# AIGC-Audio/AudioGPT

Hardware: AMD Instinct MI355X
Metric: generated audio-seconds/sec (10s clip, 100 DDIM steps) [3 independent batches of 8 prompts in flight per GPU] (higher is better)
Workload: dtype bf16x3; 1 GPU; Make-An-Audio T2A batch=8/GPU, 100 DDIM steps, CFG 1.5, UNet+VAE+HiFi-GAN(16k), fp32 storage, bf16x3-split MFMA (hi/lo, fp32 accumulate; meets the fp32 parity gates); prompts_per_gpu=8, ddim_steps=100, mel_frames=624, hipgraph=True, batches_in_flight=3, cfg_lanes=1, concurrency_hint=3, parallelism=prompt-sharded x1 (RCCL bcast cond / gather wav)

## Files before the change

### audiogpt_amd/csrc/igemm_dma.hip

```cpp
#include "igemm_epilogue.h"

#include <cstdio>
#include <cstdlib>

namespace maa {

namespace {

constexpr int NT = 256;

template <int BM, int BN, int WGM, int WGN, int NS, int TERMS>
__global__ __launch_bounds__(NT) void igemm_dma_kernel(const IGemm p, int ntiles, int Nb) {
    constexpr int WTM = BM / WGM, WTN = BN / WGN;
    constexpr int MI = WTM / 32, NI = WTN / 32;
    constexpr int ROWS = BM + BN;
    constexpr int STAGE = ROWS * 128;
    constexpr int IPW = ROWS / 32;
    static_assert(WGM * WGN == 4 && BM % 32 == 0 && BN % 32 == 0 && NS >= 2, "tile");
    static_assert((NS - 2) * IPW <= 63, "vmcnt field");
    extern __shared__ __attribute__((aligned(1024))) char smem[];

    const int tid = threadIdx.x;
    const int lane = tid & 63, wid = tid >> 6;
    const int bid = xcd_contiguous((int)blockIdx.x, (int)gridDim.x);
    const int nt = bid % ntiles, mt = bid / ntiles;
    const int m0 = mt * BM, n0 = nt * BN;

    const int Ctot = p.C1;
    const int rpb = p.Hout * p.Wout;
    const int Hlim = p.Hin << p.up, Wlim = p.Win << p.up;
    const int taps = p.KH * p.KW;
    const char* zero = reinterpret_cast<const char*>(p.zeros);

    bool is_a[IPW];
    int a_b[IPW], a_iy0[IPW], a_ix0[IPW];
    const char* a_slot[IPW];
    const char* src[IPW];
    bool ok[IPW];
#pragma unroll
    for (int j = 0; j < IPW; ++j) {
        const int row = 8 * (wid * IPW + j) + (lane >> 3);
        const int slot = (lane & 7) ^ ((row >> 1) & 7);
        is_a[j] = 8 * (wid * IPW + j) < BM;
        a_b[j] = -1;
        a_iy0[j] = a_ix0[j] = 0;
        a_slot[j] = reinterpret_cast<const char*>(p.a1) + slot * 16;
        src[j] = zero;
        ok[j] = false;
        if (is_a[j]) {
            const int m = m0 + row;
            if (m < p.M) {
                const int b = m / rpb;
                const int rem = m - b * rpb;
                const int oy = rem / p.Wout;
                a_b[j] = b;
                a_iy0[j] = oy * p.sh - p.ph;
                a_ix0[j] = (rem - oy * p.Wout) * p.sw - p.pw;
            }
        } else {
            const int n = n0 + row - BM;
            ok[j] = n < Nb;
            src[j] = reinterpret_cast<const char*>(p.b) + (long long)(ok[j] ? n : 0) * p.ldb * 4 + slot * 16;
        }
    }
    auto set_tap = [&](int tap) {
        const int ky = tap / p.KW, kx = tap - ky * p.KW;
#pragma unroll
        for (int j = 0; j < IPW; ++j)
            if (is_a[j]) {
                int iy = a_iy0[j] + ky * p.dh, ix = a_ix0[j] + kx * p.dw;
                const bool v = a_b[j] >= 0 && iy >= 0 && iy < Hlim && ix >= 0 && ix < Wlim;
                iy >>= p.up;
                ix >>= p.up;
                const long long off = v ? ((long long)a_b[j] * p.Hin + iy) * p.Win + ix : 0;
                ok[j] = v;
                src[j] = a_slot[j] + off * p.lda1 * 4;
            }
    };
    int g_tap = 0, g_ci = 0;
    bool past = false;
    auto issue = [&](int stage) {
        char* sbase = smem + stage * STAGE + wid * (IPW * 1024);
        const int k0 = g_tap * Ctot + g_ci;
#pragma unroll
        for (int j = 0; j < IPW; ++j) {
            const int off = is_a[j] ? g_ci : k0;
            const bool live = ok[j] && !past && (is_a[j] || k0 < p.K);
            const char* g = live ? src[j] + (long long)off * 4 : zero;
            __builtin_amdgcn_global_load_lds((gptr_t)g, (lptr_t)(sbase + j * 1024), 16, 0, 0);
        }
        g_ci += BK;
        if (g_ci >= Ctot) {
            g_ci = 0;
            ++g_tap;
            if (g_tap < taps)
                set_tap(g_tap);
            else
                past = true;
        }
    };

    f32x16 acc[MI][NI];
#pragma unroll
    for (int i = 0; i < MI; ++i)
#pragma unroll
        for (int j = 0; j < NI; ++j)
#pragma unroll
            for (int r = 0; r < 16; ++r) acc[i][j][r] = 0.f;

    const int wm = wid / WGN, wn = wid - wm * WGN;
    const int lrow = lane & 31, lk = lane >> 5;
    const int swz = (lrow >> 1) & 7;
    const int a_row = (wm * WTM + lrow) * 128, b_row = (BM + wn * WTN + lrow) * 128;
    int slot_off[2][2];
#pragma unroll
    for (int pl = 0; pl < 2; ++pl)
#pragma unroll
        for (int ks = 0; ks < 2; ++ks) slot_off[pl][ks] = ((pl * 4 + ks * 2 + lk) ^ swz) << 4;

    auto compute = [&](int stage) {
        const char* base = smem + stage * STAGE;
        constexpr int G = MI * NI == 1 ? 2 : 1;
#pragma unroll
        for (int k0 = 0; k0 < 2; k0 += G) {
            bf16x8 ah[G][MI], bh[G][NI], al[G][MI], bl[G][NI];
#pragma unroll
            for (int g = 0; g < G; ++g) {
                const int ks = k0 + g;
#pragma unroll
                for (int i = 0; i < MI; ++i)
                    if constexpr (TERMS == 3) al[g][i] = *reinterpret_cast<const bf16x8*>(base + a_row + i * 4096 + slot_off[1][ks]);
#pragma unroll
                for (int j = 0; j < NI; ++j) bh[g][j] = *reinterpret_cast<const bf16x8*>(base + b_row + j * 4096 + slot_off[0][ks]);
#pragma unroll
                for (int i = 0; i < MI; ++i) ah[g][i] = *reinterpret_cast<const bf16x8*>(base + a_row + i * 4096 + slot_off[0][ks]);
#pragma unroll
                for (int j = 0; j < NI; ++j)
                    if constexpr (TERMS == 3) bl[g][j] = *reinterpret_cast<const bf16x8*>(base + b_row + j * 4096 + slot_off[1][ks]);
            }
            __builtin_amdgcn_sched_barrier(0);
#pragma unroll
            for (int g = 0; g < G; ++g) {
                if constexpr (TERMS == 3) {
#pragma unroll
                    for (int i = 0; i < MI; ++i)
#pragma unroll
                        for (int j = 0; j < NI; ++j)
                            acc[i][j] = __builtin_amdgcn_mfma_f32_32x32x16_bf16(al[g][i], bh[g][j], acc[i][j], 0, 0, 0);
#pragma unroll
                    for (int i = 0; i < MI; ++i)
#pragma unroll
                        for (int j = 0; j < NI; ++j)
                            acc[i][j] = __builtin_amdgcn_mfma_f32_32x32x16_bf16(ah[g][i], bl[g][j], acc[i][j], 0, 0, 0);
                }
#pragma unroll
                for (int i = 0; i < MI; ++i)
#pragma unroll
                    for (int j = 0; j < NI; ++j)
                        acc[i][j] = __builtin_amdgcn_mfma_f32_32x32x16_bf16(ah[g][i], bh[g][j], acc[i][j], 0, 0, 0);
            }
        }
    };

    const int nchunks = (p.K + BK - 1) / BK;
    set_tap(0);
#pragma unroll
    for (int s = 0; s < NS - 1; ++s) issue(s);
    int st = 0, st_fill = NS - 1;
    for (int c = 0; c < nchunks; ++c) {
        wait_vmcnt<(NS - 2) * IPW>();
        __builtin_amdgcn_s_barrier();
        issue(st_fill);
        compute(st);
        st = st + 1 == NS ? 0 : st + 1;
        st_fill = st_fill + 1 == NS ? 0 : st_fill + 1;
    }
    wait_vmcnt<0>();

    igemm_epilogue<MI, NI>(p, acc, m0 + wm * WTM, n0 + wn * WTN, lrow, lk, 0, Nb, rpb);
}

template <int BM, int BN, int WGM, int WGN, int NS, int TERMS>
void launch_terms(const Ctx& ctx, const IGemm& p, int Nb) {
    const int ncols = p.N * (p.geglu ? 2 : 1);
    const int mtiles = (p.M + BM - 1) / BM, ntiles = (ncols + BN - 1) / BN;
    dim3 grid((unsigned)((long long)mtiles * ntiles));
    constexpr size_t lds = (size_t)NS * (BM + BN) * 128;
    auto kern = igemm_dma_kernel<BM, BN, WGM, WGN, NS, TERMS>;
    ensure_dynamic_lds(reinterpret_cast<const void*>(kern), ctx.device, (int)lds);
    hipLaunchKernelGGL(kern, grid, dim3(NT), lds, ctx.stream, p, ntiles, Nb);
}

template <int BM, int BN, int WGM, int WGN, int NS>
void launch_one(const Ctx& ctx, const IGemm& p, int Nb) {
    if (ctx.dtype == 2)
        launch_terms<BM, BN, WGM, WGN, NS, 1>(ctx, p, Nb);
    else
        launch_terms<BM, BN, WGM, WGN, NS, 3>(ctx, p, Nb);
}

}

bool igemm_dma_takes(const Ctx&, const IGemm& p, IGemmPlan& pl) {
    const long long ncols = (long long)p.N * (p.geglu ? 2 : 1);
    if (pl.cfg == 2 && p.K >= 1024 && ((p.M + 127) / 128) * ((ncols + 63) / 64) >= 448) pl.cfg = 1;
    pl.engine = IGemmPlan::DMA;
    return true;
}

void launch_igemm_dma(const Ctx& ctx, const IGemm& p, const IGemmPlan& pl) {
    const int cfg = pl.cfg, Nb = pl.Nb;
    const long long ncols = (long long)p.N * (p.geglu ? 2 : 1);
    int ns = cfg == 2 ? 2 : cfg == 1 ? 3 : 2;
    if (cfg == 2) {
        const long long tiles = (long long)((p.M + 63) / 64) * ((ncols + 63) / 64);
        if (tiles * 2 < 5LL * device_cu_count(ctx.device)) ns = 3;
    }
    switch (cfg) {
        case 0:
            launch_one<128, 128, 2, 2, 2>(ctx, p, Nb);
            break;
        case 1:
            launch_one<128, 64, 2, 2, 3>(ctx, p, Nb);
            break;
        default:
            if (ns >= 4) launch_one<64, 64, 2, 2, 4>(ctx, p, Nb);
            else if (ns == 3) launch_one<64, 64, 2, 2, 3>(ctx, p, Nb);
            else launch_one<64, 64, 2, 2, 2>(ctx, p, Nb);
            break;
    }
}

}
```

### audiogpt_amd/csrc/igemm_epilogue.h

```cpp
#pragma once
#include "igemm_device.h"
#include "maa_internal.h"

namespace maa {

__device__ __forceinline__ float fast_erff(float x) {
    const float t = fminf(fabsf(x), 4.0f);
    const float s = t * t;
    float r = -5.654105860e-04f;
    r = fmaf(r, s, 4.923277665e-03f);
    r = fmaf(r, s, -2.671638510e-02f);
    r = fmaf(r, s, 1.128036441e-01f);
    r = fmaf(r, s, -3.761234978e-01f);
    r = fmaf(r, s, 1.128379127e+00f);
    const float small = r * t;
    float q = 1.330939039e-05f;
    q = fmaf(q, t, -3.175720346e-04f);
    q = fmaf(q, t, 3.436867598e-03f);
    q = fmaf(q, t, -2.262198592e-02f);
    q = fmaf(q, t, 1.033189800e-01f);
    q = fmaf(q, t, 6.390933195e-01f);
    q = fmaf(q, t, 1.125925949e+00f);
    q = fmaf(q, t, 7.569686250e-04f);
    const float large = 1.0f - __builtin_amdgcn_exp2f(q * -1.4426950408889634f);
    return copysignf(t < 1.0f ? small : large, x);
}

__device__ __forceinline__ void settle(float& x) { asm volatile("" : "+v"(x)); }

__device__ __forceinline__ void store_split_pair(float* row, int n, float v) {
    const __bf16 h = (__bf16)v;
    const unsigned hb = __builtin_bit_cast(unsigned short, h);
    const __bf16 l = (__bf16)(v - __builtin_bit_cast(float, hb << 16));
    const unsigned lb = __builtin_bit_cast(unsigned short, l);
    const bool even = (n & 1) == 0;
    const unsigned mine = even ? lb : hb;
    const unsigned theirs = (unsigned)__builtin_amdgcn_update_dpp(0, (int)mine, 0xB1, 0xF, 0xF, false);
    unsigned* o = reinterpret_cast<unsigned*>(reinterpret_cast<unsigned short*>(row) + (n >> 5) * 64 + ((n & 31) & ~1) + (even ? 0 : 32));
    *o = even ? (hb | (theirs << 16)) : (theirs | (lb << 16));
}

template <int MI, int NI, bool PAIR, bool RSEL>
__device__ __forceinline__ void igemm_epilogue_impl(const IGemm& p, f32x16 (&acc)[MI][NI], int m_base, int n_base,
                                                    int lrow, int lk, long long coff, int Nb, int rpb) {
    float* cp = p.c + coff;
    const float* resp = p.res ? p.res + coff : nullptr;
    if (p.geglu) {
        if constexpr (NI % 2 == 0) {
#pragma unroll
            for (int i = 0; i < MI; ++i)
#pragma unroll
                for (int j = 0; j < NI; j += 2) {
                    const int cpk = n_base + j * 32 + lrow;
                    const int ncol = (cpk >> 6) * 32 + lrow;
                    if (cpk + 32 < Nb && ncol < p.N) {
                        float bv = p.bias ? p.bias[cpk] : 0.f;
                        float bg = p.bias ? p.bias[cpk + 32] : 0.f;
                        settle(bv);
                        settle(bg);
                        float outv[16];
#pragma unroll
                        for (int r = 0; r < 16; ++r) {
                            const float val = acc[i][j][r] * p.alpha + bv;
                            const float g = acc[i][j + 1][r] * p.alpha + bg;
                            const float gl = 0.5f * g * (1.f + fast_erff(g * 0.70710678118654752440f));
                            outv[r] = val * gl;
                        }
#pragma unroll
                        for (int r = 0; r < 16; ++r) {
                            const int m = m_base + i * 32 + (r & 3) + 8 * (r >> 2) + 4 * lk;
                            if (m < p.M) {
                                if (p.c_split)
                                    store_split_pair(cp + (long long)m * p.ldc, ncol, outv[r]);
                                else
                                    cp[(long long)m * p.ldc + ncol] = outv[r];
                            }
                        }
                    }
                }
        }
        return;
    }
#pragma unroll
    for (int i = 0; i < MI; ++i) {
        const int mb = m_base + i * 32;
        const int b0 = (mb < p.M ? mb : p.M - 1) / rpb;
        const int nextb = (b0 + 1) * rpb;
#pragma unroll
        for (int j = 0; j < NI; ++j) {
            const int n = n_base + j * 32 + lrow;
            if (n < p.N) {
                float bias = p.bias ? p.bias[n] : 0.f;
                float ra[16], rs[16], cv[16];
                long long mc[16];
#pragma unroll
                for (int r = 0; r < 16; ++r) {
                    const int m = mb + (r & 3) + 8 * (r >> 2) + 4 * lk;
                    mc[r] = m < p.M ? m : p.M - 1;
                    ra[r] = rs[r] = cv[r] = 0.f;
                }
                if (p.rowadd) {
                    if constexpr (RSEL) {
                        const float* ra0 = p.rowadd + (long long)b0 * p.ld_rowadd + n;
#pragma unroll
                        for (int r = 0; r < 16; ++r) ra[r] = ra0[mc[r] < nextb ? 0 : p.ld_rowadd];
                    } else {
#pragma unroll
                        for (int r = 0; r < 16; ++r) ra[r] = p.rowadd[(long long)((int)mc[r] / rpb) * p.ld_rowadd + n];
                    }
                }
                if (resp) {
#pragma unroll
                    for (int r = 0; r < 16; ++r) rs[r] = resp[mc[r] * p.ldr + n];
                }
                if (p.accumulate && !p.c_split) {
#pragma unroll
                    for (int r = 0; r < 16; ++r) cv[r] = cp[mc[r] * p.ldc + n];
                }
                settle(bias);
#pragma unroll
                for (int r = 0; r < 16; ++r) {
                    settle(ra[r]);
                    settle(rs[r]);
                    settle(cv[r]);
                }
                float outv[16];
#pragma unroll
                for (int r = 0; r < 16; ++r) {
                    float v = acc[i][j][r] * p.alpha + bias;
                    if (p.rowadd) v += ra[r];
                    if (resp) v += rs[r];
                    outv[r] = v;
                }
                if (p.act != 0) {
#pragma unroll
                    for (int r = 0; r < 16; ++r) {
                        float v = outv[r];
                        if (p.act == 1) v = tanhf(v);
                        else if (p.act == 2) v = fmaxf(v, 0.f);
                        else if (p.act == 3) v = 0.5f * v * (1.f + fast_erff(v * 0.70710678118654752440f));
                        else if (p.act == 4) v = v > 0.f ? v : v * p.act_slope;
                        outv[r] = v;
                    }
                }
#pragma unroll
                for (int r = 0; r < 16; ++r) {
                    float v = outv[r] * p.out_scale;
                    if (p.accumulate && !p.c_split) v += cv[r];
                    outv[r] = v;
                }
                if constexpr (PAIR) {
                    const bool even = (lrow & 1) == 0;
#pragma unroll
                    for (int rp = 0; rp < 8; ++rp) {
                        const float keep = even ? outv[2 * rp] : outv[2 * rp + 1];
                        const float give = even ? outv[2 * rp + 1] : outv[2 * rp];
                        const float got = __builtin_bit_cast(float, __builtin_amdgcn_update_dpp(0, __builtin_bit_cast(int, give), 0xB1, 0xF, 0xF, false));
                        const int r = 2 * rp + (even ? 0 : 1);
                        const int m = mb + (r & 3) + 8 * (r >> 2) + 4 * lk;
                        if (m < p.M) {
                            const f32x2 v2 = even ? f32x2{keep, got} : f32x2{got, keep};
                            *reinterpret_cast<f32x2*>(cp + (long long)m * p.ldc + (n & ~1)) = v2;
                        }
                    }
                } else {
#pragma unroll
                    for (int r = 0; r < 16; ++r) {
                        const int m = mb + (r & 3) + 8 * (r >> 2) + 4 * lk;
                        if (m < p.M) {
                            if (p.c_split)
                                store_split_pair(cp + (long long)m * p.ldc, n, outv[r]);
                            else
                                cp[(long long)m * p.ldc + n] = outv[r];
                            if (p.c2) {
                                const float w = outv[r] > 0.f ? outv[r] : outv[r] * p.c2_slope;
                                store_split_pair(p.c2 + coff + (long long)m * p.ldc2, n, w);
                            }
                        }
                    }
                }
            }
        }
    }
}

template <int MI, int NI>
__device__ __forceinline__ void igemm_epilogue(const IGemm& p, f32x16 (&acc)[MI][NI], int m_base, int n_base, int lrow,
                                               int lk, long long coff, int Nb, int rpb) {
    const bool pair = !p.geglu && !p.c_split && p.c2 == nullptr && (p.N & 1) == 0 && (p.ldc & 1) == 0 && (coff & 1) == 0 &&
                      (reinterpret_cast<uintptr_t>(p.c) & 7) == 0;
    const bool rsel = !(p.rowadd && rpb < 32);
    if (pair && rsel)
        igemm_epilogue_impl<MI, NI, true, true>(p, acc, m_base, n_base, lrow, lk, coff, Nb, rpb);
    else if (pair)
        igemm_epilogue_impl<MI, NI, true, false>(p, acc, m_base, n_base, lrow, lk, coff, Nb, rpb);
    else if (rsel)
        igemm_epilogue_impl<MI, NI, false, true>(p, acc, m_base, n_base, lrow, lk, coff, Nb, rpb);
    else
        igemm_epilogue_impl<MI, NI, false, false>(p, acc, m_base, n_base, lrow, lk, coff, Nb, rpb);
}

}
```

### audiogpt_amd/csrc/maa_internal.h

```cpp
#pragma once
#include <hip/hip_runtime.h>

#include <cstdint>
#include <cstdio>
#include <map>
#include <stdexcept>
#include <string>
#include <vector>

namespace maa {

struct Error : std::runtime_error {
    using std::runtime_error::runtime_error;
};
void set_last_error(const std::string& s);

#define MAA_HIP(expr)                                                                              \
    do {                                                                                           \
        hipError_t _e = (expr);                                                                    \
        if (_e != hipSuccess)                                                                      \
            throw ::maa::Error(std::string(#expr) + ": " + hipGetErrorString(_e));                 \
    } while (0)
#define MAA_CHECK(cond, msg)                                                                       \
    do {                                                                                           \
        if (!(cond)) throw ::maa::Error(std::string("check failed: ") + #cond + " -- " + (msg));   \
    } while (0)

class Arena {
public:
    ~Arena();
    void reserve(size_t bytes);
    void reset() { off_ = 0; run_high_ = 0; }
    size_t mark() const { return off_; }
    void release(size_t m) { off_ = m; }
    float* alloc_f(size_t n_floats);
    size_t capacity() const { return cap_; }
    const void* base() const { return base_; }
    size_t high_water() const { return high_; }
    size_t mark_high() const { return run_high_; }
    bool dry = false;

private:
    char* base_ = nullptr;
    size_t cap_ = 0, off_ = 0, high_ = 0, run_high_ = 0;
};

struct ProfRow {
    std::string name;
    long long launches = 0;
    double ms = 0.0, flops = 0.0, bytes = 0.0;
};
class Profiler {
public:
    ~Profiler();
    struct Pending {
        std::string name;
        double flops, bytes;
        hipEvent_t e0, e1;
    };
    hipEvent_t get_event();
    std::vector<Pending> pending;
    std::vector<hipEvent_t> pool;
    size_t next = 0;
    int detail = 0;
    std::vector<ProfRow> collect(hipStream_t stream);
};
struct Ctx;
struct ProfScope {
    ProfScope(const Ctx& ctx, const char* name, double flops, double bytes);
    ~ProfScope();
    const Ctx* ctx_ = nullptr;
    size_t idx_ = 0;
};

void ensure_dynamic_lds(const void* kernel, int device, int bytes);
int device_cu_count(int device);

struct DevSlab {
    void* p = nullptr;
    size_t cap = 0;
    ~DevSlab();
    void* get(size_t bytes, hipStream_t stream);
    DevSlab() = default;
    DevSlab(const DevSlab&) = delete;
    DevSlab& operator=(const DevSlab&) = delete;
};

struct StepGraph {
    std::vector<unsigned long long> key;
    hipGraph_t graph = nullptr;
    hipGraphExec_t exec = nullptr;
    void clear();
    ~StepGraph() { clear(); }
    StepGraph() = default;
    StepGraph(const StepGraph&) = delete;
    StepGraph& operator=(const StepGraph&) = delete;
};

struct Tuning {
    std::string dma2;
    std::string pp, pp1;
    int pp_s_narrow = 2, pp_s_wide = 4;
    bool up2 = true;
    bool pp_tile_major = false;
    bool op_presplit = false;
    bool no_dma = false;
    int halo = 2;
    bool cfg_shared = true;
    bool gn_two_pass = false;
    void load();
};

struct Ctx {
    Ctx() = default;
    Ctx(const Ctx&) = delete;
    Ctx& operator=(const Ctx&) = delete;
    ~Ctx();
    Ctx* side = nullptr;
    hipEvent_t ev_fork = nullptr, ev_join = nullptr;
    int concurrency = -1;
    bool kept_full() const { return concurrency >= 3; }
    int cfg_split = -1;
    bool split_cfg() const { return cfg_split < 0 ? !kept_full() : cfg_split != 0; }
    Tuning tune;
    StepGraph ddim_graph;
    DevSlab sampler_scratch;
    DevSlab encode_scratch;
    StepGraph plms_graph;
    DevSlab plms_ring;
    StepGraph ddpm_graph;
    DevSlab ddpm_tab;
    DevSlab ddpm_scratch;
    DevSlab split_scratch;
    Profiler* prof = nullptr;
    float* zeros = nullptr;
    int device = 0;
    hipStream_t stream = nullptr;
    mutable Arena ws;
    int dtype = 0;
};

Ctx& side_lane(Ctx& ctx);

struct IGemm {
    const float* a1 = nullptr;
    const float* a2 = nullptr;
    int lda1 = 0, lda2 = 0;
    int C1 = 0, C2 = 0;
    int Hin = 1, Win = 1, Hout = 1, Wout = 1;
    int KH = 1, KW = 1, sh = 1, sw = 1, ph = 0, pw = 0, dh = 1, dw = 1;
    int up = 0;
    int a_split = 0;
    int a_act = 0;
    float a_slope = 0.f;
    const float* b = nullptr;
    int ldb = 0;
    int b_nk = 0;
    int b_split = 0;
    int M = 0, N = 0, K = 0;
    int Z = 1, zin = 1;
    long long a_so = 0, a_si = 0, b_so = 0, b_si = 0, c_so = 0, c_si = 0;
    float alpha = 1.f;
    const float* bias = nullptr;
    const float* rowadd = nullptr;
    int ld_rowadd = 0;
    const float* res = nullptr;
    int ldr = 0;
    int geglu = 0;
    int act = 0;
    float act_slope = 0.f;
    float out_scale = 1.f;
    int accumulate = 0;
    int c_split = 0;
    float* c = nullptr;
    int ldc = 0;
    float* c2 = nullptr;
    int ldc2 = 0;
    float c2_slope = 1.f;
    const float* zeros = nullptr;
};
struct IGemmPlan {
    enum Engine { F32, BF16_REG, DMA, DMA2, PP, PP1 } engine = F32;
    int cfg = 0;
    int bn = 0;
    int S = 1;
    int Nb = 0;
    bool fast = false;
    size_t slab_floats = 0;
};
IGemmPlan igemm_plan(const Ctx& ctx, const IGemm& p);
void launch_igemm(const Ctx& ctx, const IGemm& p);
int choose_tile(long long M, long long N, int Z, bool bf16, int mode = 0);
int fit_slices(int nchunks, int S);
void launch_igemm_f32(const Ctx& ctx, const IGemm& p, const IGemmPlan& pl);
void launch_igemm_bf16_reg(const Ctx& ctx, const IGemm& p, const IGemmPlan& pl);
bool igemm_dma_takes(const Ctx& ctx, const IGemm& p, IGemmPlan& pl);
void launch_igemm_dma(const Ctx& ctx, const IGemm& p, const IGemmPlan& pl);
bool igemm_dma2_takes(const Ctx& ctx, const IGemm& p, IGemmPlan& pl);
void launch_igemm_dma2(const Ctx& ctx, const IGemm& p, const IGemmPlan& pl, float* part);
bool igemm_pp_takes(const Ctx& ctx, const IGemm& p, IGemmPlan& pl);
void launch_igemm_pp(const Ctx& ctx, const IGemm& p, const IGemmPlan& pl, float* part);
bool igemm_pp1_takes(const Ctx& ctx, const IGemm& p, IGemmPlan& pl);
void launch_igemm_pp1(const Ctx& ctx, const IGemm& p, const IGemmPlan& pl, float* part);
void launch_splitk_reduce(const Ctx& ctx, const IGemm& p, const float* part, int S, int tiles, int ntiles, int Nb, int BM,
                          int BN, int WGN, int MI, int NI, int NTH);

void launch_groupnorm(Ctx& ctx, const float* x1, int ld1, int C1, const float* x2, int ld2, int C2, int B, int HW,
                      int groups, const float* gamma, const float* beta, float eps, int silu, float* out,
                      int out_split = 0, float* raw_split = nullptr);
void launch_layernorm(const Ctx& ctx, const float* x, long long rows, int C, const float* gamma, const float* beta,
                      float eps, float* out, int out_split = 0);
bool launch_igemm_pp_up2(const Ctx& ctx, const IGemm& p, int Nb, long long b_phase);
bool launch_narrow_conv3x3(const Ctx& ctx, const float* a_split, int lda, int B, int H, int W, int C, const float* w4, const float* bias,
                           int N, float* out_nchw);
void launch_pixel_shuffle2(const Ctx& ctx, const float* planes, int B, int H, int W, int C, float* out);
void launch_split32_pack(const Ctx& ctx, const float* x, long long rows, int C, float* out, float slope = 1.f);
void launch_split32_unpack(const Ctx& ctx, const float* x, long long rows, int C, float* out);
bool launch_flash_attention(const Ctx& ctx, const float* q, int ldq, int hsq, const float* k, int ldk, int hsk,
                            const float* v, int ldv, int hsv, int B, int heads, int dh, int Nq, int Nk, float alpha,
                            float* out, int ldo, int out_split = 0, int causal = 0);
bool flash_attention_covers(const Ctx& ctx, int dh);
void launch_softmax(const Ctx& ctx, float* s, long long rows, int cols, int ld, int causal_nq = 0);

void launch_timestep_embedding(const Ctx& ctx, const float* t, int B, int dim, float* out);
void launch_silu(const Ctx& ctx, const float* x, long long n, float* out);
void launch_add(const Ctx& ctx, const float* a, const float* b, long long n, float* out);
void launch_nchw_to_nhwc(const Ctx& ctx, const float* x, int B, int C, int HW, float* out);
void launch_nhwc_to_nchw(const Ctx& ctx, const float* x, int B, int C, int HW, float* out, int ld_in);
void launch_avgpool2(const Ctx& ctx, const float* x, int B, int H, int W, int C, float* out);
void launch_upsample2(const Ctx& ctx, const float* x, int B, int H, int W, int C, float* out);
void launch_dup_half(const Ctx& ctx, const float* x, long long n, float* out);
void split_check(int H, int W, int kh, int kw, int sh, int sw);
int split_crops(int H, int W, int kh, int kw, int sh, int sw);
void launch_split_unfold(const Ctx& ctx, const float* x, int nB, int C, int H, int W, int kh, int kw, int sh, int sw, float* out);
void launch_split_norm(const Ctx& ctx, const float* wT, int H, int W, int kh, int kw, int sh, int sw, float* norm);
void launch_split_fold(const Ctx& ctx, const float* e, const float* wT, const float* norm, int nB, int C, int H, int W, int kh,
                       int kw, int sh, int sw, float* out);
void launch_repeat_rows(const Ctx& ctx, const float* src, long long rows, long long len, int rep, float* dst);
void launch_scale(const Ctx& ctx, const float* x, long long n, float s, float* out);
void launch_ddim_update(const Ctx& ctx, const float* x, const float* eps_u, const float* eps_c, float scale,
                        const float* coef, long long n, float* x_prev, float* pred_x0, int* step = nullptr);
void launch_ddim_prepare(const Ctx& ctx, const float* x, const float* concat, int B, int nB, long long per,
                         long long per_c, const float* tab_t, const float* tab_coef, const int* step, float* xin,
                         float* cur_t, float* cur_coef, const float* mask = nullptr, const float* x0 = nullptr,
                         const float* noise_q = nullptr, int S = 0, const float* emb_tab = nullptr, int emb_w = 0,
                         float* cur_emb = nullptr, int n_t = 0);
void launch_ddim_step(const Ctx& ctx, const float* xin, long long per, long long per_in, const float* eps_u, const float* eps_c,
                      float scale, const float* coef, long long n, float* x_prev, const float* noise_p, float temperature, int S,
                      float* log_x, float* log_x0, int* step);
void launch_ldm_plms_step(const Ctx& ctx, const float* xin, long long per, long long per_in, const float* eps_u, const float* eps_c,
                          float scale, const float* coef, long long n, float* x_prev, float* ring, int S, float* log_x, float* log_x0,
                          int* step);
void launch_ldm_plms_euler_mid(const Ctx& ctx, float* xin, long long per, long long per_in, int B, int nB, const float* eps_u,
                               const float* eps_c, float scale, const float* coef, float* x_save, float* e_keep, const float* tab_t,
                               float* cur_t, const float* emb_tab, int emb_w, float* cur_emb, int n_t = 0);
void launch_ldm_plms_euler_final(const Ctx& ctx, const float* eps_u, const float* eps_c, float scale, const float* coef, long long n,
                                 float* x, const float* e_keep, float* log_x, float* log_x0, int* step);
constexpr int DDPM_TAB_W = 9;
void launch_ddpm_step(const Ctx& ctx, const float* xin, long long per, long long per_in, const float* eps_u, const float* eps_c,
                      float scale, const float* coef, const float* tab, long long n, float* x_prev, const float* noise_p, int start,
                      bool clip, const float* mask, const float* x0, const float* noise_q, float* log_x, float* log_x0, int* step);
// ... 72 lines not shown
```

### audiogpt_amd/csrc/runtime.cpp

```cpp
#include "maa_internal.h"

#include <mutex>

#include <cstdlib>
#include <cstring>

extern char** environ;

namespace maa {

static thread_local std::string g_last_error;
void set_last_error(const std::string& s) { g_last_error = s; }
const char* last_error_cstr() { return g_last_error.c_str(); }

Arena::~Arena() {
    if (base_) (void)hipFree(base_);
}
void Arena::reserve(size_t bytes) {
    if (bytes <= cap_) return;
    if (base_) MAA_HIP(hipFree(base_));
    base_ = nullptr;
    cap_ = 0;
    MAA_HIP(hipMalloc(reinterpret_cast<void**>(&base_), bytes));
    cap_ = bytes;
}
float* Arena::alloc_f(size_t n_floats) {
    const size_t bytes = (n_floats * sizeof(float) + 255) / 256 * 256;
    const size_t at = off_;
    off_ += bytes;
    if (off_ > high_) high_ = off_;
    if (off_ > run_high_) run_high_ = off_;
    if (dry) return reinterpret_cast<float*>(static_cast<uintptr_t>(0x1000) + at);
    if (off_ > cap_) throw Error("workspace arena exhausted (" + std::to_string(off_) + " > " + std::to_string(cap_) + ")");
    return reinterpret_cast<float*>(base_ + at);
}

DevSlab::~DevSlab() {
    if (p) (void)hipFree(p);
}
void* DevSlab::get(size_t bytes, hipStream_t stream) {
    if (bytes > cap) {
        if (p) {
            MAA_HIP(hipStreamSynchronize(stream));
            MAA_HIP(hipFree(p));
            p = nullptr;
            cap = 0;
        }
        const size_t want = bytes + bytes / 4;
        MAA_HIP(hipMalloc(&p, want));
        cap = want;
    }
    return p;
}

Profiler::~Profiler() {
    for (hipEvent_t e : pool) (void)hipEventDestroy(e);
}
hipEvent_t Profiler::get_event() {
    if (next == pool.size()) {
        hipEvent_t e;
        MAA_HIP(hipEventCreate(&e));
        pool.push_back(e);
    }
    return pool[next++];
}
std::vector<ProfRow> Profiler::collect(hipStream_t stream) {
    MAA_HIP(hipStreamSynchronize(stream));
    std::map<std::string, ProfRow> agg;
    for (auto& p : pending) {
        float ms = 0.f;
        MAA_HIP(hipEventElapsedTime(&ms, p.e0, p.e1));
        ProfRow& r = agg[p.name];
        r.name = p.name;
        r.launches += 1;
        r.ms += ms;
        r.flops += p.flops;
        r.bytes += p.bytes;
    }
    pending.clear();
    next = 0;
    std::vector<ProfRow> out;
    for (auto& kv : agg) out.push_back(kv.second);
    return out;
}
ProfScope::ProfScope(const Ctx& ctx, const char* name, double flops, double bytes) {
    if (!ctx.prof || ctx.ws.dry) return;
    hipStreamCaptureStatus st = hipStreamCaptureStatusNone;
    if (hipStreamIsCapturing(ctx.stream, &st) != hipSuccess || st != hipStreamCaptureStatusNone) return;
    ctx_ = &ctx;
    Profiler::Pending p;
    p.name = name;
    p.flops = flops;
    p.bytes = bytes;
    p.e0 = ctx.prof->get_event();
    p.e1 = ctx.prof->get_event();
    (void)hipEventRecord(p.e0, ctx.stream);
    idx_ = ctx.prof->pending.size();
    ctx.prof->pending.push_back(p);
}
ProfScope::~ProfScope() {
    if (ctx_) (void)hipEventRecord(ctx_->prof->pending[idx_].e1, ctx_->stream);
}

const HostTensor& get(const StateDict& sd, const std::string& name) {
    auto it = sd.find(name);
    if (it == sd.end()) throw Error("missing weight tensor: " + name);
    return it->second;
}
bool has(const StateDict& sd, const std::string& name) { return sd.find(name) != sd.end(); }

void Tuning::load() {
#ifdef MAA_NO_TUNING
    return;
#endif
    auto get_s = [](const char* name) {
        const char* e = std::getenv(name);
        return std::string(e ? e : "");
    };
    dma2 = get_s("MAA_DMA2");
    pp = get_s("MAA_PP");
    pp1 = get_s("MAA_PP1");
    pp_s_narrow = 2;
    pp_s_wide = 4;
    const std::string pss = get_s("MAA_PP_S");
    if (!pss.empty()) std::sscanf(pss.c_str(), "%d,%d", &pp_s_narrow, &pp_s_wide);
    if (pp_s_narrow < 1) pp_s_narrow = 1;
    if (pp_s_wide < 1) pp_s_wide = 1;
    pp_tile_major = get_s("MAA_PP_TILE_MAJOR") == "1";
    up2 = get_s("MAA_UP2") != "0";
    cfg_shared = get_s("MAA_CFG_SHARED") != "0";
    const std::string ps = get_s("MAA_OP_PRESPLIT");
    op_presplit = !ps.empty() && ps[0] == '1';
    no_dma = !get_s("MAA_NO_DMA").empty();
    const std::string hs = get_s("MAA_HALO");
    halo = hs == "off" ? 0 : hs == "single" ? 1 : 2;
    gn_two_pass = get_s("MAA_GN_TWO_PASS") == "1";
    if (!dma2.empty() && dma2 != "off") {
        int cfg = 0, ns = 4, pipe = 1, S = 1, kmin = 0, kmax = 0;
        const int k = std::sscanf(dma2.c_str(), "%d,%d,%d,%d,%d,%d", &cfg, &ns, &pipe, &S, &kmin, &kmax);
        if (k < 4 || cfg != 0 || ns != 4 || pipe != 1 || S < 1) {
            const std::string bad = dma2;
            dma2.clear();
            throw Error("MAA_DMA2=\"" + bad + "\": expected \"off\" or \"0,4,1,S[,kmin[,kmax]]\" (the split-K engine keeps one "
                        "instantiation: tile 0, 4 stages, pipelined; S = K slices)");
        }
    }
}

Ctx::~Ctx() {
    if (side) {
        (void)hipStreamSynchronize(side->stream);
        (void)hipStreamDestroy(side->stream);
        side->stream = nullptr;
        delete side->prof;
        side->prof = nullptr;
        delete side;
    }
    if (ev_fork) (void)hipEventDestroy(ev_fork);
    if (ev_join) (void)hipEventDestroy(ev_join);
}
Ctx& side_lane(Ctx& ctx) {
    if (!ctx.side) {
        hipStream_t s = nullptr;
        MAA_HIP(hipStreamCreateWithFlags(&s, hipStreamNonBlocking));
        Ctx* sd = new Ctx;
        sd->stream = s;
        sd->device = ctx.device;
        sd->zeros = ctx.zeros;
        ctx.side = sd;
        MAA_HIP(hipEventCreateWithFlags(&ctx.ev_fork, hipEventDisableTiming));
        MAA_HIP(hipEventCreateWithFlags(&ctx.ev_join, hipEventDisableTiming));
    }
    ctx.side->tune = ctx.tune;
    ctx.side->dtype = ctx.dtype;
    ctx.side->concurrency = ctx.kept_full() ? 3 : 1;
    return *ctx.side;
}

void StepGraph::clear() {
    if (exec) (void)hipGraphExecDestroy(exec);
    if (graph) (void)hipGraphDestroy(graph);
    exec = nullptr;
    graph = nullptr;
    key.clear();
}

namespace {
std::mutex g_launch_mu;
std::map<std::pair<const void*, int>, int> g_lds_attr;
std::map<int, int> g_cus;
}

void ensure_dynamic_lds(const void* kernel, int device, int bytes) {
    std::lock_guard<std::mutex> lk(g_launch_mu);
    int& have = g_lds_attr[{kernel, device}];
    if (have >= bytes) return;
    MAA_HIP(hipFuncSetAttribute(kernel, hipFuncAttributeMaxDynamicSharedMemorySize, bytes));
    have = bytes;
}

int device_cu_count(int device) {
    std::lock_guard<std::mutex> lk(g_launch_mu);
    int& c = g_cus[device];
    if (!c) {
        hipDeviceProp_t prop;
        MAA_HIP(hipGetDeviceProperties(&prop, device));
        c = prop.multiProcessorCount;
    }
    return c;
}

WeightStore::~WeightStore() {
    for (void* p : bufs_) (void)hipFree(p);
}
float* WeightStore::upload(const std::vector<float>& host) {
    void* d = nullptr;
    const size_t bytes = host.size() * sizeof(float);
    MAA_HIP(hipMalloc(&d, bytes ? bytes : 4));
    if (bytes) MAA_HIP(hipMemcpy(d, host.data(), bytes, hipMemcpyHostToDevice));
    bufs_.push_back(d);
    bytes_ += bytes;
    return static_cast<float*>(d);
}
float* WeightStore::vec(const StateDict& sd, const std::string& name) {
    const HostTensor& t = get(sd, name);
    return upload(std::vector<float>(t.data, t.data + t.numel()));
}

static int pad32(int n) { return (n + 31) / 32 * 32; }

static inline unsigned short f2bf(float f) {
    unsigned u;
    std::memcpy(&u, &f, 4);
    u += 0x7fffu + ((u >> 16) & 1u);
    return (unsigned short)(u >> 16);
}
static inline float bf2f(unsigned short h) {
    const unsigned u = (unsigned)h << 16;
    float f;
    std::memcpy(&f, &u, 4);
    return f;
}
void* WeightStore::upload_raw(const void* host, size_t bytes) {
    void* d = nullptr;
    MAA_HIP(hipMalloc(&d, bytes ? bytes : 4));
    if (bytes) MAA_HIP(hipMemcpy(d, host, bytes, hipMemcpyHostToDevice));
    bufs_.push_back(d);
    bytes_ += bytes;
    return d;
}

void WeightStore::finish(PackedW& pw, const std::vector<float>& kn, bool bf16_ok) {
    if (nk_ && bf16_ok) {
        MAA_CHECK(pw.K % 32 == 0, "split32 weights need K % 32 == 0");
        const int ldk = pw.K;
        std::vector<unsigned short> t((size_t)pw.Npad * ldk * 2, 0);
        for (int k = 0; k < pw.K; ++k)
            for (int n = 0; n < pw.Npad; ++n) {
                const float w = kn[(size_t)k * pw.Npad + n];
                const unsigned short hi = f2bf(w);
                const size_t at = (size_t)n * ldk * 2 + (size_t)(k >> 5) * 64 + (k & 31);
                t[at] = hi;
                t[at + 32] = f2bf(w - bf2f(hi));
            }
        pw.w = static_cast<float*>(upload_raw(t.data(), t.size() * sizeof(unsigned short)));
        pw.ld = ldk;
        pw.nk = 1;
        pw.split = 1;
        return;
    }
    if (!nk_) {
        pw.w = upload(kn);
        pw.ld = pw.Npad;
        pw.nk = 0;
        return;
    }
    const int Kp = (pw.K + 3) / 4 * 4;
    std::vector<float> t((size_t)pw.Npad * Kp, 0.f);
    for (int k = 0; k < pw.K; ++k)
        for (int n = 0; n < pw.Npad; ++n) t[(size_t)n * Kp + k] = kn[(size_t)k * pw.Npad + n];
    pw.w = upload(t);
    pw.ld = Kp;
    pw.nk = 1;
}

PackedW WeightStore::pack_conv(const StateDict& sd, const std::string& wname, const std::string& bname, int KH,
                               int KW) {
    const HostTensor& w = get(sd, wname);
    MAA_CHECK(w.shape.size() >= 2, wname);
// ... 172 lines not shown
```

Before: 135.9 audio-seconds/sec.

## Add linear-GEMM fast path with specialized epilogues in igemm DMA kernel

Adds a LINEAR template path for 1x1, unstrided, unpadded convolutions and plain linear layers. It replaces the per-tap im2col address setup with simple pointer advances and computes the tile index with a reciprocal multiply instead of a division. It also adds specialized epilogues (plain paired f32x2 stores via DPP, bf16 hi/lo split stores, and fused GEGLU) with full-tile and residual variants, so common epilogues skip the generic path's bookkeeping. Setting MAA_EPI=generic restores the old path. The cost is more template instantiations, code size and register pressure, and added risk in the correctness of the new store paths.

```diff
diff --git a/audiogpt_amd/csrc/igemm_dma.hip b/audiogpt_amd/csrc/igemm_dma.hip
--- a/audiogpt_amd/csrc/igemm_dma.hip
+++ b/audiogpt_amd/csrc/igemm_dma.hip
@@ -9,8 +9,8 @@
 
 constexpr int NT = 256;
 
-template <int BM, int BN, int WGM, int WGN, int NS, int TERMS>
-__global__ __launch_bounds__(NT) void igemm_dma_kernel(const IGemm p, int ntiles, int Nb) {
+template <int BM, int BN, int WGM, int WGN, int NS, int TERMS, bool LINEAR = false, Epi EPI = Epi::GENERIC>
+__global__ __launch_bounds__(NT) void igemm_dma_kernel(const IGemm p, int ntiles, int Nb, unsigned ntiles_rcp) {
     constexpr int WTM = BM / WGM, WTN = BN / WGN;
     constexpr int MI = WTM / 32, NI = WTN / 32;
     constexpr int ROWS = BM + BN;
@@ -23,7 +23,18 @@
     const int tid = threadIdx.x;
     const int lane = tid & 63, wid = tid >> 6;
     const int bid = xcd_contiguous((int)blockIdx.x, (int)gridDim.x);
-    const int nt = bid % ntiles, mt = bid / ntiles;
+    int nt, mt;
+    if constexpr (LINEAR) {
+        mt = (int)__umulhi((unsigned)bid, ntiles_rcp);
+        nt = bid - mt * ntiles;
+        if (nt >= ntiles) {
+            nt -= ntiles;
+            ++mt;
+        }
+    } else {
+        nt = bid % ntiles;
+        mt = bid / ntiles;
+    }
     const int m0 = mt * BM, n0 = nt * BN;
 
     const int Ctot = p.C1;
@@ -37,30 +48,45 @@
     const char* a_slot[IPW];
     const char* src[IPW];
     bool ok[IPW];
-#pragma unroll
-    for (int j = 0; j < IPW; ++j) {
-        const int row = 8 * (wid * IPW + j) + (lane >> 3);
-        const int slot = (lane & 7) ^ ((row >> 1) & 7);
-        is_a[j] = 8 * (wid * IPW + j) < BM;
-        a_b[j] = -1;
-        a_iy0[j] = a_ix0[j] = 0;
-        a_slot[j] = reinterpret_cast<const char*>(p.a1) + slot * 16;
-        src[j] = zero;
-        ok[j] = false;
-        if (is_a[j]) {
-            const int m = m0 + row;
-            if (m < p.M) {
-                const int b = m / rpb;
-                const int rem = m - b * rpb;
-                const int oy = rem / p.Wout;
-                a_b[j] = b;
-                a_iy0[j] = oy * p.sh - p.ph;
-                a_ix0[j] = (rem - oy * p.Wout) * p.sw - p.pw;
-            }
-        } else {
-            const int n = n0 + row - BM;
-            ok[j] = n < Nb;
-            src[j] = reinterpret_cast<const char*>(p.b) + (long long)(ok[j] ? n : 0) * p.ldb * 4 + slot * 16;
+    int adv[IPW];
+    if constexpr (LINEAR) {
+#pragma unroll
+        for (int j = 0; j < IPW; ++j) {
+            const int row = 8 * (wid * IPW + j) + (lane >> 3);
+            const int slot = (lane & 7) ^ ((row >> 1) & 7);
+            const bool a = 8 * (wid * IPW + j) < BM;
+            const int idx = a ? m0 + row : n0 + row - BM;
+            const bool live = idx < (a ? p.M : Nb);
+            const char* base = reinterpret_cast<const char*>(a ? p.a1 : p.b);
+            src[j] = live ? base + (long long)idx * (a ? p.lda1 : p.ldb) * 4 + slot * 16 : zero;
+            adv[j] = live ? BK * 4 : 0;
+        }
+    } else {
+#pragma unroll
+        for (int j = 0; j < IPW; ++j) {
+            const int row = 8 * (wid * IPW + j) + (lane >> 3);
+            const int slot = (lane & 7) ^ ((row >> 1) & 7);
+            is_a[j] = 8 * (wid * IPW + j) < BM;
+            a_b[j] = -1;
+            a_iy0[j] = a_ix0[j] = 0;
+            a_slot[j] = reinterpret_cast<const char*>(p.a1) + slot * 16;
+            src[j] = zero;
+            ok[j] = false;
+            if (is_a[j]) {
+                const int m = m0 + row;
+                if (m < p.M) {
+                    const int b = m / rpb;
+                    const int rem = m - b * rpb;
+                    const int oy = rem / p.Wout;
+                    a_b[j] = b;
+                    a_iy0[j] = oy * p.sh - p.ph;
+                    a_ix0[j] = (rem - oy * p.Wout) * p.sw - p.pw;
+                }
+            } else {
+                const int n = n0 + row - BM;
+                ok[j] = n < Nb;
+                src[j] = reinterpret_cast<const char*>(p.b) + (long long)(ok[j] ? n : 0) * p.ldb * 4 + slot * 16;
+            }
         }
     }
     auto set_tap = [&](int tap) {
@@ -79,8 +105,24 @@
     };
     int g_tap = 0, g_ci = 0;
     bool past = false;
+    int left = (p.K + BK - 1) / BK;
     auto issue = [&](int stage) {
         char* sbase = smem + stage * STAGE + wid * (IPW * 1024);
+        if constexpr (LINEAR) {
+#pragma unroll
+            for (int j = 0; j < IPW; ++j) {
+                __builtin_amdgcn_global_load_lds((gptr_t)src[j], (lptr_t)(sbase + j * 1024), 16, 0, 0);
+                src[j] += adv[j];
+            }
+            if (--left == 0) {
+#pragma unroll
+                for (int j = 0; j < IPW; ++j) {
+                    src[j] = zero;
+                    adv[j] = 0;
+                }
+            }
+            return;
+        }
         const int k0 = g_tap * Ctot + g_ci;
 #pragma unroll
         for (int j = 0; j < IPW; ++j) {
@@ -163,7 +205,7 @@
     };
 
     const int nchunks = (p.K + BK - 1) / BK;
-    set_tap(0);
+    if constexpr (!LINEAR) set_tap(0);
 #pragma unroll
     for (int s = 0; s < NS - 1; ++s) issue(s);
     int st = 0, st_fill = NS - 1;
@@ -177,26 +219,46 @@
     }
     wait_vmcnt<0>();
 
-    igemm_epilogue<MI, NI>(p, acc, m0 + wm * WTM, n0 + wn * WTN, lrow, lk, 0, Nb, rpb);
-}
-
-template <int BM, int BN, int WGM, int WGN, int NS, int TERMS>
+    if constexpr (EPI == Epi::GENERIC)
+        igemm_epilogue<MI, NI>(p, acc, m0 + wm * WTM, n0 + wn * WTN, lrow, lk, 0, Nb, rpb);
+    else
+        igemm_epilogue_fast<MI, NI, EPI>(p, acc, m0 + wm * WTM, n0 + wn * WTN, lrow, lk, Nb);
+}
+
+template <int BM, int BN, int WGM, int WGN, int NS, int TERMS, bool LINEAR, Epi EPI>
 void launch_terms(const Ctx& ctx, const IGemm& p, int Nb) {
     const int ncols = p.N * (p.geglu ? 2 : 1);
     const int mtiles = (p.M + BM - 1) / BM, ntiles = (ncols + BN - 1) / BN;
     dim3 grid((unsigned)((long long)mtiles * ntiles));
     constexpr size_t lds = (size_t)NS * (BM + BN) * 128;
-    auto kern = igemm_dma_kernel<BM, BN, WGM, WGN, NS, TERMS>;
+    auto kern = igemm_dma_kernel<BM, BN, WGM, WGN, NS, TERMS, LINEAR, EPI>;
     ensure_dynamic_lds(reinterpret_cast<const void*>(kern), ctx.device, (int)lds);
-    hipLaunchKernelGGL(kern, grid, dim3(NT), lds, ctx.stream, p, ntiles, Nb);
+    const unsigned long long rcp = (1ULL << 32) / (unsigned)ntiles;
+    hipLaunchKernelGGL(kern, grid, dim3(NT), lds, ctx.stream, p, ntiles, Nb, (unsigned)(rcp > 0xFFFFFFFFULL ? 0xFFFFFFFFULL : rcp));
+}
+
+template <int BM, int BN, int WGM, int WGN, int NS, bool LINEAR, Epi EPI>
+void launch_kind(const Ctx& ctx, const IGemm& p, int Nb) {
+    if (ctx.dtype == 2)
+        launch_terms<BM, BN, WGM, WGN, NS, 1, LINEAR, EPI>(ctx, p, Nb);
+    else
+        launch_terms<BM, BN, WGM, WGN, NS, 3, LINEAR, EPI>(ctx, p, Nb);
+}
+
+bool igemm_is_linear(const IGemm& p) {
+    return p.KH == 1 && p.KW == 1 && p.sh == 1 && p.sw == 1 && p.ph == 0 && p.pw == 0 && p.up == 0 && p.a2 == nullptr && p.C2 == 0 &&
+           p.K == p.C1 && p.Hin == p.Hout && p.Win == p.Wout;
 }
 
 template <int BM, int BN, int WGM, int WGN, int NS>
 void launch_one(const Ctx& ctx, const IGemm& p, int Nb) {
-    if (ctx.dtype == 2)
-        launch_terms<BM, BN, WGM, WGN, NS, 1>(ctx, p, Nb);
-    else
-        launch_terms<BM, BN, WGM, WGN, NS, 3>(ctx, p, Nb);
+    const Epi kind = ctx.tune.epi_generic || !igemm_is_linear(p) ? Epi::GENERIC : igemm_epi_kind(p);
+    if (kind == Epi::PLAIN) return launch_kind<BM, BN, WGM, WGN, NS, true, Epi::PLAIN>(ctx, p, Nb);
+    if (kind == Epi::SPLIT) return launch_kind<BM, BN, WGM, WGN, NS, true, Epi::SPLIT>(ctx, p, Nb);
+    if constexpr ((BN / WGN / 32) % 2 == 0) {
+        if (kind == Epi::GEGLU) return launch_kind<BM, BN, WGM, WGN, NS, true, Epi::GEGLU>(ctx, p, Nb);
+    }
+    launch_kind<BM, BN, WGM, WGN, NS, false, Epi::GENERIC>(ctx, p, Nb);
 }
 
 }
diff --git a/audiogpt_amd/csrc/igemm_epilogue.h b/audiogpt_amd/csrc/igemm_epilogue.h
--- a/audiogpt_amd/csrc/igemm_epilogue.h
+++ b/audiogpt_amd/csrc/igemm_epilogue.h
@@ -28,16 +28,19 @@
 
 __device__ __forceinline__ void settle(float& x) { asm volatile("" : "+v"(x)); }
 
-__device__ __forceinline__ void store_split_pair(float* row, int n, float v) {
+__device__ __forceinline__ unsigned split_pair_word(bool even, float v) {
     const __bf16 h = (__bf16)v;
     const unsigned hb = __builtin_bit_cast(unsigned short, h);
     const __bf16 l = (__bf16)(v - __builtin_bit_cast(float, hb << 16));
     const unsigned lb = __builtin_bit_cast(unsigned short, l);
-    const bool even = (n & 1) == 0;
     const unsigned mine = even ? lb : hb;
     const unsigned theirs = (unsigned)__builtin_amdgcn_update_dpp(0, (int)mine, 0xB1, 0xF, 0xF, false);
+    return even ? (hb | (theirs << 16)) : (theirs | (lb << 16));
+}
+__device__ __forceinline__ void store_split_pair(float* row, int n, float v) {
+    const bool even = (n & 1) == 0;
     unsigned* o = reinterpret_cast<unsigned*>(reinterpret_cast<unsigned short*>(row) + (n >> 5) * 64 + ((n & 31) & ~1) + (even ? 0 : 32));
-    *o = even ? (hb | (theirs << 16)) : (theirs | (lb << 16));
+    *o = split_pair_word(even, v);
 }
 
 template <int MI, int NI, bool PAIR, bool RSEL>
@@ -200,4 +203,156 @@
         igemm_epilogue_impl<MI, NI, false, false>(p, acc, m_base, n_base, lrow, lk, coff, Nb, rpb);
 }
 
-}
+enum class Epi : int { GENERIC = 0, PLAIN = 1, SPLIT = 2, GEGLU = 3 };
+
+inline Epi igemm_epi_kind(const IGemm& p) {
+    const bool pitches = p.ldc > 0 && p.ldc < (1 << 24) && p.ldr >= 0 && p.ldr < (1 << 24);
+    if (!pitches || p.Z != 1 || p.M <= 0 || p.alpha != 1.f || p.out_scale != 1.f || p.rowadd || p.act != 0 || p.accumulate || p.c2)
+        return Epi::GENERIC;
+    if (p.geglu) return p.res ? Epi::GENERIC : Epi::GEGLU;
+    if (p.c_split) return (p.N & 1) == 0 ? Epi::SPLIT : Epi::GENERIC;
+    const bool pair = (p.N & 1) == 0 && (p.ldc & 1) == 0 && (reinterpret_cast<uintptr_t>(p.c) & 7) == 0;
+    return pair ? Epi::PLAIN : Epi::GENERIC;
+}
+
+__device__ __forceinline__ constexpr unsigned frag_row(int r) { return (unsigned)((r & 3) + 8 * (r >> 2)); }
+
+template <int MI, int NI, Epi KIND, bool FULL, bool RES>
+__device__ __forceinline__ void igemm_epilogue_fast_body(const IGemm& p, f32x16 (&acc)[MI][NI], int mb0, int nb0, int lrow, int lk,
+                                                         int Nb) {
+    const bool even = (lrow & 1) == 0;
+    const unsigned ldc = (unsigned)p.ldc, ldr = (unsigned)p.ldr;
+    const unsigned lane_f32 = 4u * lk * ldc + lrow;
+    const unsigned lane_pair = (4u * lk + (even ? 0u : 1u)) * ldc + (lrow & ~1);
+    const unsigned lane_split = 4u * lk * ldc + (lrow >> 1) + (even ? 0u : 16u);
+    const unsigned lane_res = 4u * lk * ldr + lrow;
+    if constexpr (KIND == Epi::GEGLU) {
+        static_assert(NI % 2 == 0, "GEGLU pairs a value block with a gate block");
+#pragma unroll
+        for (int i = 0; i < MI; ++i) {
+            const int mb = mb0 + i * 32;
+            if (!FULL && mb >= p.M) break;
+#pragma unroll
+            for (int j = 0; j < NI; j += 2) {
+                const int cb = nb0 + j * 32, ob = (cb >> 6) * 32;
+                const int cpk = cb + lrow;
+                if (FULL || (cpk + 32 < Nb && ob + lrow < p.N)) {
+                    float bv = p.bias ? p.bias[cpk] : 0.f;
+                    float bg = p.bias ? p.bias[cpk + 32] : 0.f;
+                    settle(bv);
+                    settle(bg);
+                    float outv[16];
+#pragma unroll
+                    for (int r = 0; r < 16; ++r) {
+                        const float val = acc[i][j][r] + bv;
+                        const float g = acc[i][j + 1][r] + bg;
+                        const float gl = 0.5f * g * (1.f + fast_erff(g * 0.70710678118654752440f));
+                        outv[r] = val * gl;
+                    }
+                    float* blk = p.c + ((long long)mb * ldc + ob);
+                    if (p.c_split) {
+#pragma unroll
+                        for (int r = 0; r < 16; ++r) {
+                            const unsigned w = split_pair_word(even, outv[r]);
+                            if (FULL || mb + (int)frag_row(r) + 4 * lk < p.M) reinterpret_cast<unsigned*>(blk)[lane_split + frag_row(r) * ldc] = w;
+                        }
+                    } else {
+#pragma unroll
+                        for (int r = 0; r < 16; ++r)
+                            if (FULL || mb + (int)frag_row(r) + 4 * lk < p.M) blk[lane_f32 + frag_row(r) * ldc] = outv[r];
+                    }
+                }
+            }
+        }
+    } else {
+#pragma unroll
+        for (int i = 0; i < MI; ++i) {
+            const int mb = mb0 + i * 32;
+            if (!FULL && mb >= p.M) break;
+            const unsigned last = (unsigned)(p.M - 1 - mb);
+#pragma unroll
+            for (int j = 0; j < NI; ++j) {
+                const int nb = nb0 + j * 32;
+                if (FULL || nb + lrow < p.N) {
+                    float bias = p.bias ? p.bias[nb + lrow] : 0.f;
+                    float rs[16];
+                    if constexpr (RES) {
+                        const float* rb = p.res + ((long long)mb * ldr + nb);
+#pragma unroll
+                        for (int r = 0; r < 16; ++r) {
+                            if constexpr (FULL) {
+                                rs[r] = rb[lane_res + frag_row(r) * ldr];
+                            } else {
+                                const unsigned row = frag_row(r) + 4u * lk;
+                                rs[r] = rb[(row < last ? row : last) * ldr + lrow];
+                            }
+                        }
+                    }
+                    settle(bias);
+                    float outv[16];
+#pragma unroll
+                    for (int r = 0; r < 16; ++r) {
+                        float v = acc[i][j][r] + bias;
+                        if constexpr (RES) {
+                            settle(rs[r]);
+                            v += rs[r];
+                        }
+                        outv[r] = v;
+                    }
+                    float* blk = p.c + ((long long)mb * ldc + nb);
+                    if constexpr (KIND == Epi::PLAIN) {
+#pragma unroll
+                        for (int rp = 0; rp < 8; ++rp) {
+                            const float keep = even ? outv[2 * rp] : outv[2 * rp + 1];
+                            const float give = even ? outv[2 * rp + 1] : outv[2 * rp];
+                            const float got = __builtin_bit_cast(float, __builtin_amdgcn_update_dpp(0, __builtin_bit_cast(int, give), 0xB1, 0xF, 0xF, false));
+                            const f32x2 v2 = even ? f32x2{keep, got} : f32x2{got, keep};
+                            if (FULL || mb + (int)frag_row(2 * rp) + 4 * lk + (even ? 0 : 1) < p.M)
+                                *reinterpret_cast<f32x2*>(blk + (lane_pair + frag_row(2 * rp) * ldc)) = v2;
+                        }
+                    } else {
+#pragma unroll
+                        for (int r = 0; r < 16; ++r) {
+                            const unsigned w = split_pair_word(even, outv[r]);
+                            if (FULL || mb + (int)frag_row(r) + 4 * lk < p.M) reinterpret_cast<unsigned*>(blk)[lane_split + frag_row(r) * ldc] = w;
+                        }
+                    }
+                }
+            }
+        }
+    }
+}
+
+template <int MI, int NI, Epi KIND>
+__device__ __forceinline__ void igemm_epilogue_fast(const IGemm& p, f32x16 (&acc)[MI][NI], int m_base, int n_base, int lrow, int lk,
+                                                    int Nb) {
+    static_assert(KIND != Epi::GENERIC, "the generic kind is igemm_epilogue");
+    const int mb0 = __builtin_amdgcn_readfirstlane(m_base), nb0 = __builtin_amdgcn_readfirstlane(n_base);
+    if (mb0 >= p.M) return;
+    bool full = mb0 + MI * 32 <= p.M;
+    if constexpr (KIND == Epi::GEGLU) {
+        const int cpk = nb0 + (NI - 2) * 32 + 31;
+        if (nb0 + 32 >= Nb) return;
+        full = full && cpk + 32 < Nb && (cpk >> 6) * 32 + 31 < p.N;
+        if (full)
+            igemm_epilogue_fast_body<MI, NI, KIND, true, false>(p, acc, mb0, nb0, lrow, lk, Nb);
+        else
+            igemm_epilogue_fast_body<MI, NI, KIND, false, false>(p, acc, mb0, nb0, lrow, lk, Nb);
+    } else {
+        if (nb0 >= p.N) return;
+        full = full && nb0 + NI * 32 <= p.N;
+        if (p.res) {
+            if (full)
+                igemm_epilogue_fast_body<MI, NI, KIND, true, true>(p, acc, mb0, nb0, lrow, lk, Nb);
+            else
+                igemm_epilogue_fast_body<MI, NI, KIND, false, true>(p, acc, mb0, nb0, lrow, lk, Nb);
+        } else {
+            if (full)
+                igemm_epilogue_fast_body<MI, NI, KIND, true, false>(p, acc, mb0, nb0, lrow, lk, Nb);
+            else
+                igemm_epilogue_fast_body<MI, NI, KIND, false, false>(p, acc, mb0, nb0, lrow, lk, Nb);
+        }
+    }
+}
+
+}
diff --git a/audiogpt_amd/csrc/maa_internal.h b/audiogpt_amd/csrc/maa_internal.h
--- a/audiogpt_amd/csrc/maa_internal.h
+++ b/audiogpt_amd/csrc/maa_internal.h
@@ -107,6 +107,7 @@
     bool no_dma = false;
     int halo = 2;
     bool cfg_shared = true;
+    bool epi_generic = false;
     bool gn_two_pass = false;
     void load();
 };
diff --git a/audiogpt_amd/csrc/runtime.cpp b/audiogpt_amd/csrc/runtime.cpp
--- a/audiogpt_amd/csrc/runtime.cpp
+++ b/audiogpt_amd/csrc/runtime.cpp
@@ -135,6 +135,7 @@
     const std::string hs = get_s("MAA_HALO");
     halo = hs == "off" ? 0 : hs == "single" ? 1 : 2;
     gn_two_pass = get_s("MAA_GN_TWO_PASS") == "1";
+    epi_generic = get_s("MAA_EPI") == "generic";
     if (!dma2.empty() && dma2 != "off") {
         int cfg = 0, ns = 4, pipe = 1, S = 1, kmin = 0, kmax = 0;
         const int k = std::sscanf(dma2.c_str(), "%d,%d,%d,%d,%d,%d", &cfg, &ns, &pipe, &S, &kmin, &kmax);
```

New measurement: 140.6 audio-seconds/sec, median of 6. +3.4%, better.
